# jyjblrd/Low-Cost-Mocap

Measured on AMD Instinct MI355X. Metric: triangulated 3D markers/sec at 8 cams x 16 markers, higher is better.
Workload: dtype f64

## Files before the change

### low-cost-mocap_amd/csrc/frame_bb.hip

```cpp
#include "mocap_device.hpp"
#include "kernels.hpp"
#include <cstdlib>
#include "frame_common.hpp"
#include "bb_fold.hpp"

namespace mocap {

constexpr int kBBThreads = 256;
constexpr int kBBWaves = kBBThreads / 64;
constexpr int kBBRecs = kBBThreads + 64;
constexpr int bb_cw(int C) { return C <= 8 ? 1 : 2; }
constexpr uint32_t bb_rec_bytes(int CW) { return 24u + 8u * (uint32_t)CW; }

constexpr int bb_wg_per_cu(int RL) { return RL == 48 ? 5 : 4; }
constexpr size_t kBBCacheEntry = 4;
constexpr int kBBLdsSlack = 1024;
struct BBLayout {
  size_t bxy, bxy_nx, cnt_nx, bt, rbound, seedkey, slot_key, claimw, recs, rpk, scr, scr_bytes, goff, gcnt, outslot, boff, bnb, seedgh, slot_g, cnt,
      misc, bpl, nh, hits, act, root_blob, root_cam, nact, bnl, bv, pkbase, seen, bcache, total;
  int ncache;
  __host__ __device__ static size_t al(size_t x, size_t a) { return (x + a - 1) / a * a; }
  __host__ __device__ BBLayout(int C, int M, int R, int CW, int wg_per_cu) {
    size_t o = 0;
    auto take = [&](size_t bytes, size_t a) {
// ... 553 lines not shown
        }
        const bool flag = lane < Mi && !((claimed >> lane) & 1ull);
        const unsigned long long mask = __ballot(flag);
        const int pos = __popcll(mask & ((1ull << lane) - 1ull));
        if (flag) {
          const int rr = n_roots + pos;
          if (rr < R) {
            root_cam[rr] = (uint8_t)i;
            root_blob[rr] = (uint8_t)lane;
          }
        }
        int slot = n_new;
        for (unsigned long long mm = mask; mm; slot++) {
          const int jb = __ffsll((long long)mm) - 1;
          mm &= mm - 1;
          if (lane == slot) {
            nr_cam = i;
            nr_blob = jb;
          }
        }
        n_roots += __popcll(mask);
        if (n_roots > R) {
          over = true;
          n_roots = R;
        }
      }
      if (lane == 0) {
        if (over) misc[MI_STATUS] |= MOCAP_ST_ROOT_OVERFLOW_;
        misc[MI_NROOTS] = n_roots;
      }
    } else {
      float om = 0.0f;
      for (int i = tid - 64; i < C * M; i += T - 64) {
        const int c = i / M, k = i - c * M;
        if (k < cnt[c]) {
          const float2 v = bxy[i];
          om = fmaxf(om, fmaxf(fabsf(v.x), fabsf(v.y)));
          double Bc[10];
          dlt_contribution(Bc, cv.pq(PERK ? 12 * (c * C + c) : 12 * c), (double)v.x, (double)v.y);
#pragma unroll
          for (int e = 0; e < 10; e++) bt[(size_t)i * 10 + e] = Bc[e];
        }
      }
      if (om > 0.0f) atomicMax(&misc[MI_OMAX], __float_as_int(om));
      if (tid == 64) {
        const int it = q_add(&p.q.counters[QC_NEXT_FRAME], 1);
        misc[MI_NEXT] = it < frame_count(p) ? it : -1;
      }
    }
    bb_prio<kPrioPhase>();
    __syncthreads();
    if (pre) {
      const int n_new = misc[MI_NROOTS] - n0;
      for (int idx = tid; idx < n_new * C; idx += T) {
        const int q = idx / C, c = idx - q * C;
        const int r = n0 + q, ps = bnl[q];
        if (c > (int)root_cam[r]) {
          const int n = nh_s[(size_t)ps * C + c];
          nh[(size_t)r * C + c] = (uint8_t)n;
          const uint8_t* src = hits_s + ((size_t)ps * C + c) * M;
          uint8_t* dst = hits + ((size_t)r * C + c) * M;
          for (int t = 0; t < n; t++) dst[t] = src[t];
        }
      }
      __syncthreads();
    }

    fresh_tid();
    const int nroots = misc[MI_NROOTS];
    for (int r = tid; r < nroots; r += T) {
      const int rc = root_cam[r];
      unsigned long long total = 1;
      int views = 1, na = 0;
      bool over = false;
      Packed<CW> pkb;
      pkb.clear();
      pkb.set(rc, root_blob[r]);
      uint32_t sm = 1u << rc;
      for (int c = rc + 1; c < C; c++) {
        const unsigned n = nh[(size_t)r * C + c];
        if (n > 1) act[(size_t)r * C + na++] = (uint8_t)c;
        if (n == 1) pkb.set(c, hits[((size_t)r * C + c) * M]);
        if (n) {
          sm |= 1u << c;
          views++;
          total *= n;
          if (total > (unsigned long long)p.G_cap) {
            over = true;
            total = 1;
          }
        }
      }
      if (over) atomicOr(&misc[MI_STATUS], MOCAP_ST_CAND_OVERFLOW_);
      nact[r] = (uint8_t)na;
      bv[r] = (uint8_t)views;
#pragma unroll
      for (int k = 0; k < CW; k++) pkbase[(size_t)r * CW + k] = pkb.w[k];
      if (PERK) seen[r] = (uint16_t)sm;
      rbound[r] = kInfBits;
      const uint32_t g = (views > 1 && !over) ? (uint32_t)total : 0u;
      gcnt[r] = g;
      {
        const uint8_t* a = act + (size_t)r * C;
        uint32_t pl = 1, nb = 1;
        int nl = 0;
        for (int k = 0; k < na; k++) nb *= nh[(size_t)r * C + a[k]];
        if (over) nb = 1;
        while (nl < na && (pl < (uint32_t)p.bb_pl_min || (pl < (uint32_t)p.bb_pl && nb > (uint32_t)p.bb_nb_max))) {
          const uint32_t n = nh[(size_t)r * C + a[nl++]];
          uint32_t dummy;
          pl *= n;
          divmod_small(nb, n, nb, dummy);
        }
        bpl[r] = (uint16_t)pl;
        bnl[r] = (uint8_t)nl;
        bnb[r] = g ? nb : 0u;
        seedkey[r] = 0ull;
        seedgh[r] = 0xFFFFFFFFu;
      }
    }
    for (int s = tid; s < W * RS; s += T) {
      slot_key[s] = ~0ull;
      slot_g[s] = 0xFFFFFFFFu;
    }
    if (tid == 0) misc[MI_BBCTR] = misc[MI_BBCTR2] = 0;
    __syncthreads();
    if (wave == 0) bb_prio<kPrioSerial>();
    if (wave == 0) {
      uint32_t carry = 0, bcarry = 0;
      int slots = 0;
      for (int base = 0; base < nroots; base += 64) {
        const int r = base + lane;
        const uint32_t g = r < nroots ? gcnt[r] : 0u;
        const uint32_t nb = r < nroots ? bnb[r] : 0u;
        const uint32_t incl = wave_inclusive_scan(g, lane);
        const uint32_t bincl = wave_inclusive_scan(nb, lane);
        const unsigned long long nz = __ballot(g != 0u);
        if (r < nroots) {
          goff[r] = carry + incl - g;
          boff[r] = bcarry + bincl - nb;
          outslot[r] = g ? slots + __popcll(nz & ((1ull << lane) - 1ull)) : -1;
        }
        carry += (uint32_t)__builtin_amdgcn_readlane((int)incl, 63);
        bcarry += (uint32_t)__builtin_amdgcn_readlane((int)bincl, 63);
        slots += __popcll(nz);
      }
      if (lane == 0) {
        goff[nroots] = carry;
        boff[nroots] = bcarry;
        misc[MI_NOUT] = slots;
        misc[MI_G] = misc[MI_STATUS] ? 0 : (int32_t)carry;
      }
    }
    bb_prio<kPrioPhase>();
    __syncthreads();
  }

  __device__ __forceinline__ void add_view(double (&B)[10], int c, uint32_t k, int j) const {
    if (PERK && j != c) {
      const float2 w = bxy[(size_t)c * M + k];
      double Bc[10];
      dlt_contribution(Bc, cv.base + 12 * ((size_t)j * cn() + c), (double)w.x, (double)w.y);
#pragma unroll
      for (int e = 0; e < 10; e++) B[e] = B[e] + Bc[e];
    } else {
      const double* t = bt + ((size_t)c * M + k) * 10;
#pragma unroll
      for (int e = 0; e < 10; e++) B[e] = B[e] + t[e];
    }
  }

  template <bool WITH_B>
  __device__ __forceinline__ int group_matrix(int r, uint32_t rem, int skip, double (&B)[10], Packed<CW>& pk) const {
    const int C = cn();
    const int rc = root_cam[r];
    const uint8_t* nhr = nh + (size_t)r * C;
    const uint8_t* hr = hits + (size_t)r * C * M;
    pk.clear();
    int v = 0, ka = 0;
    int j = 0;
    if (WITH_B) {
#pragma unroll
      for (int e = 0; e < 10; e++) B[e] = 0.0;
    }
    for (int c = 0; c < C; c++) {
      uint32_t k = 0xFFu;
      bool seen = false;
      if (c == rc) {
        k = root_blob[r];
        seen = true;
      } else if (c > rc) {
        const uint32_t n = nhr[c];
        seen = n != 0;
        if (n == 1) {
          k = hr[(size_t)c * M];
        } else if (n > 1) {
          if (ka >= skip) {
            uint32_t qd, dgt;
            if (rem < 8192u) divmod_tiny(rem, n, qd, dgt); else
            divmod_small(rem, n, qd, dgt);
            rem = qd;
            k = hr[(size_t)c * M + dgt];
          }
          ka++;
        }
      }
      if (k != 0xFFu) {
        if (WITH_B) add_view(B, c, k, j);
        v++;
        pk.set(c, k);
      }
      if (PERK) j += seen ? 1 : 0;
    }
    return v;
  }

  __device__ __forceinline__ void block_pk(int r, uint32_t gh, Packed<CW>& pk) const {
    const int C = cn();
#pragma unroll
    for (int k = 0; k < CW; k++) pk.w[k] = pkbase[(size_t)r * CW + k];
    const uint8_t* a = act + (size_t)r * C;
    const int na = nact[r];
    uint32_t rem = gh;
    for (int k = bnl[r]; k < na; k++) {
      const int c = a[k];
      const uint32_t n = nh[(size_t)r * C + c];
      uint32_t qd, dgt;
      if (rem < 8192u) divmod_tiny(rem, n, qd, dgt); else
      divmod_small(rem, n, qd, dgt);
      rem = qd;
      pk.set(c, hits[((size_t)r * C + c) * M + dgt]);
    }
  }
  __device__ __forceinline__ int block_matrix(int r, uint32_t gh, Packed<CW>& pk, double (&B)[10]) const {
    const int C = cn();
    block_pk(r, gh, pk);
#pragma unroll
    for (int ee = 0; ee < 10; ee++) B[ee] = 0.0;
    if constexpr (PERK) {
      const uint32_t sm = seen[r];
#pragma unroll CT > 0 ? CT : 1
      for (int c = 0; c < C; c++) {
        const uint32_t k = pk.get(c);
        if (k != 0xFFu) add_view(B, c, k, __popc(sm & ((1u << c) - 1u)));
      }
    } else {
#pragma unroll CT > 0 ? CT : 1
      for (int c = 0; c < C; c++) {
        const uint32_t k = pk.get(c);
        const double* t = bt + (size_t)(k != 0xFFu ? (uint32_t)c * (uint32_t)M + k : (uint32_t)C * (uint32_t)M) * 10;
#pragma unroll
        for (int ee = 0; ee < 10; ee++) B[ee] = B[ee] + t[ee];
      }
    }
    return (int)bv[r] - (int)bnl[r];
  }

  __device__ __forceinline__ int fetch_candidate(uint32_t lo, uint32_t i, int& r, uint32_t& gl, Packed<CW>& pk, double (&B)[10]) const {
    const int C = cn();
    const BRec rec = recs[lo];
    r = (int)(rec.rs & 0xFFu);
#pragma unroll
    for (int k = 0; k < CW; k++) pk.w[k] = rpk[(size_t)lo * CW + k];
    if (rec.rs >> 31) {
      gl = rec.gh;
    } else {
      uint32_t rem = i - (rec.rs >> 8);
      gl = rec.gh * (uint32_t)bpl[r] + rem;
      const uint8_t* a = act + (size_t)r * C;
      const int nl = bnl[r];
      for (int k = 0; k < nl; k++) {
        const int c = a[k];
        uint32_t qd, dgt;
        divmod_tiny(rem, nh[(size_t)r * C + c], qd, dgt);
        rem = qd;
        pk.set(c, hits[((size_t)r * C + c) * M + dgt]);
      }
    }
#pragma unroll
    for (int ee = 0; ee < 10; ee++) B[ee] = 0.0;
    if constexpr (PERK) {
      int j = 0;
#pragma unroll CT > 0 ? CT : 1
      for (int c = 0; c < C; c++) {
        const uint32_t k = pk.get(c);
        if (k != 0xFFu) add_view(B, c, k, j++);
      }
    } else {
#pragma unroll CT > 0 ? CT : 1
      for (int c = 0; c < C; c++) {
        const uint32_t k = pk.get(c);
        const double* t = bt + (size_t)(k != 0xFFu ? (uint32_t)c * (uint32_t)M + k : (uint32_t)C * (uint32_t)M) * 10;
#pragma unroll
        for (int ee = 0; ee < 10; ee++) B[ee] = B[ee] + t[ee];
      }
    }
    return bv[r];
  }

  __device__ void search(bool bound_tests) {
    fresh_tid();
    const int C = cn();
    (void)C;
    const int nroots = misc[MI_NROOTS];
    int32_t* ctr = &misc[MI_BBCTR];
    int32_t* ctr_other = &misc[MI_BBCTR2];
    const double inf = __builtin_huge_val();
    EigCut ec;
    {
      const double om = (double)__int_as_float(misc[MI_OMAX]);
      ec.p3max2 = p.p3max2;
      ec.o2slack = (1100.0 * 0x1p-46) * (om * om);
    }
    const double c0[3] = {p.bb_c0[0], p.bb_c0[1], p.bb_c0[2]};
    const uint32_t nblocks = boff[nroots];
    auto root_of_block = [&](uint32_t b_first_of_wave, uint32_t b) {
      return coop_last_le([&](int r) { return boff[r]; }, nroots, b_first_of_wave, b, lane);
    };
    auto push_block = [&](int r, uint32_t gh, const Packed<CW>& pk) {
      const uint32_t old = (uint32_t)atomicAdd(ctr, (int32_t)(((uint32_t)bpl[r] << 10) | 1u));
      const uint32_t slot = old & 0x3FFu;
      BRec rec;
      rec.gh = gh;
      rec.rs = (uint32_t)r | ((old >> 10) << 8);
      recs[slot] = rec;
#pragma unroll
      for (int k = 0; k < CW; k++) rpk[(size_t)slot * CW + k] = pk.w[k];
    };
    auto rec_start = [&](int k) { return (recs[k].rs & 0x7FFFFFFFu) >> 8; };
    auto root_y = [&](int r) {
      const int vf = bv[r];
      const double bound = __longlong_as_double((long long)rbound[r]);
      const double limit = bound * (double)(2 * vf) * (1.0 + 0x1p-40);
      const double limit_adj = fma(1.002, limit, (double)(2 * vf) * ec.o2slack);
      return p.p3max2c * limit_adj;
    };
    auto dropped = [&](int r, double s1, double tr) { return s1 * fma(2e-12, tr, root_y(r)) < 1.0; };
    if (bound_tests) {
      bb_prio<kPrioSeed>();
      int my_r = -1;
      uint32_t my_gh = 0;
      unsigned long long my_key = 0ull;
      Packed<CW> my_pk;
      my_pk.clear();
      for (uint32_t s0 = 0; s0 < nblocks; s0 += T) {
        const uint32_t b = s0 + (uint32_t)tid;
        if (s0 + (uint32_t)(wave * 64) >= nblocks) continue;
        const int r = root_of_block(s0 + (uint32_t)(wave * 64), b < nblocks ? b : nblocks - 1);
        if (b < nblocks) {
          const uint32_t gh = b - boff[r];
          double B[10], tr = 0.0;
          Packed<CW> pk;
          const int v = block_matrix(r, gh, pk, B);
          double s1d = __builtin_huge_val();
          float s1 = 0.0f;
          if (v >= 2) {
            s1d = eigcut_s1_shifted(B, c0, tr);
            s1 = (float)fmin(s1d, 3e38);
          }
          if (b < (uint32_t)ncache) bcache[b] = v >= 2 ? bb_fold_bound(s1d, tr) : bb_fold_inf();
          my_key = ((unsigned long long)__float_as_uint(s1) << 32) | (unsigned long long)(0xFFFFFFFFu - gh);
          my_r = r;
          my_gh = gh;
          my_pk = pk;
          atomicMax(&seedkey[r], my_key);
        }
      }
      __syncthreads();
      if (nblocks <= (uint32_t)T) {
        if (my_r >= 0 && seedkey[my_r] == my_key) {
          seedgh[my_r] = my_gh;
          push_block(my_r, my_gh, my_pk);
        }
      } else
      for (int r = tid; r < nroots; r += T) {
        if (bnb[r]) {
          const uint32_t gh = 0xFFFFFFFFu - (uint32_t)seedkey[r];
          seedgh[r] = gh;
          seedkey[r] = 0ull;
          Packed<CW> pk;
          block_pk(r, gh, pk);
          push_block(r, gh, pk);
        }
      }
      bb_prio<kPrioEval>();
      __syncthreads();
    }
    uint32_t b0 = 0;
    fresh_tid();
    while (true) {
      const uint32_t cv_ = (uint32_t)*ctr;
      const uint32_t ns = cv_ & 0x3FFu, ne = cv_ >> 10;
      const bool blocks_left = b0 < nblocks;
      const bool full = ns > (uint32_t)(kBBRecs - T);
      if (ns && (full || !blocks_left || ne >= (uint32_t)p.bb_flush)) {
        for (uint32_t i0 = 0; i0 < ne; i0 += T) {
          const uint32_t i = i0 + (uint32_t)tid;
          const bool have = i < ne;
          double e = inf, X[3] = {0, 0, 0};
          int r = 0;
          uint32_t gl = 0;
          uint32_t lo = 0;
          if (i0 + (uint32_t)(wave * 64) < ne)
            lo = (uint32_t)coop_last_le(rec_start, (int)ns, i0 + (uint32_t)(wave * 64), have ? i : ne - 1, lane);
          Packed<CW> pk;
          pk.clear();
          if (have) {
            double B[10];
            const int v = fetch_candidate(lo, i, r, gl, pk, B);
            auto obs_p = [&](int c, double& x, double& y) -> bool {
              const uint32_t k = pk.get(c);
              if (k == 0xFFu) return false;
              const float2 w = bxy[(size_t)c * M + k];
              x = (double)w.x;
              y = (double)w.y;
              return true;
            };
            const double bound = __longlong_as_double((long long)rbound[r]);
            solve_and_score<!PERK, true, F32R, false>(cv, B, v, obs_p, X, e, bound * (double)(2 * v) * (1.0 + 0x1p-40), ec);
#ifdef MOCAP_DEBUG_EIGCHECK
            if (!(e < inf)) {
              double B2[10], X2[3], e2;
#pragma unroll
              for (int ee = 0; ee < 10; ee++) B2[ee] = 0.0;
              int j2 = 0;
              for (int c = 0; c < C; c++) {
                const uint32_t k = pk.get(c);
                if (k != 0xFFu) add_view(B2, c, k, j2++);
              }
              solve_and_score<!PERK, true, F32R>(cv, B2, v, obs_p, X2, e2);
              atomicAdd(&p.status[p.n_frames], 1);
              if (e2 <= bound) printf("EIGCHECK candidate: root %d g %u bound %.17g true %.17g\n", r, gl, bound, e2);
            }
#endif
          }
          const bool fin = e < inf;
          const unsigned long long key = fin ? (unsigned long long)__double_as_longlong(e) : kInfBits;
          const uint32_t gword = (gl << 1) | ((e != e) ? 1u : 0u);
          const int ss = wave * RS + r;
          if (fin) atomicMin(&rbound[r], key);
          const bool want = have && (key < slot_key[ss] || (key == slot_key[ss] && gword < slot_g[ss]));
          if (__ballot(want)) {
            unsigned long long old = 0;
            if (want) old = atomicMin(&slot_key[ss], key);
            wave_lds_sync();
            const bool holder = want && slot_key[ss] == key;
            if (holder && old > key) slot_g[ss] = 0xFFFFFFFFu;
            wave_lds_sync();
            if (holder) atomicMin(&slot_g[ss], gword);
            wave_lds_sync();
            if (holder && slot_g[ss] == gword) store_winner(ss, X, pk);
          }
        }
        __syncthreads();
        if (tid == 0) *ctr = 0;
        {
          int32_t* t = ctr;
          ctr = ctr_other;
          ctr_other = t;
        }
        continue;
      }
      if (!blocks_left) break;
      const uint32_t b = b0 + (uint32_t)tid;
      const uint32_t bw = b0 + (uint32_t)(wave * 64);
      b0 += T;
      int r = 0;
      if (bw < nblocks) r = root_of_block(bw, b < nblocks ? b : nblocks - 1);
      bool do_push = false;
      uint32_t gh = 0;
      Packed<CW> pk;
      pk.clear();
      if (b < nblocks) {
        gh = b - boff[r];
        if (gh != seedgh[r]) {
          double B[10], tr;
          bool survive = true;
          if (bound_tests && b < (uint32_t)ncache) {
            survive = !bb_fold_dropped(bcache[b], root_y(r));
            if (survive) block_pk(r, gh, pk);
          } else if (bound_tests) {
            const int v = block_matrix(r, gh, pk, B);
            if (v >= 2) {
              const double s1 = eigcut_s1_shifted(B, c0, tr);
              survive = !dropped(r, s1, tr);
            }
          } else {
            block_pk(r, gh, pk);
          }
          do_push = survive;
#ifdef MOCAP_DEBUG_EIGCHECK
          if (!survive) {
            const double bound = __longlong_as_double((long long)rbound[r]);
            const uint32_t pl = bpl[r];
            for (uint32_t l = 0; l < pl; l++) {
              double B2[10], X2[3], e2 = inf;
              Packed<CW> pk2;
              const int v2 = group_matrix<true>(r, gh * pl + l, 0, B2, pk2);
              auto obs2 = [&](int c, double& x, double& y) -> bool {
                const uint32_t k = pk2.get(c);
                if (k == 0xFFu) return false;
                const float2 w = bxy[(size_t)c * M + k];
                x = (double)w.x;
                y = (double)w.y;
                return true;
              };
              solve_and_score<!PERK, true, F32R>(cv, B2, v2, obs2, X2, e2);
              atomicAdd(&p.status[p.n_frames + 1], 1);
              if (e2 <= bound) printf("EIGCHECK block: root %d block %u candidate %u bound %.17g true %.17g\n", r, gh, l, bound, e2);
            }
          }
#endif
        }
      }
      __syncthreads();
      if (do_push) push_block(r, gh, pk);
      __syncthreads();
    }
    wait_own_stores();
    __syncthreads();
  }

  __device__ __forceinline__ bool root_winner(int r, unsigned long long& kb, uint32_t& gw, int& wb) const {
    kb = ~0ull;
    gw = 0xFFFFFFFFu;
    wb = 0;
    for (int w = 0; w < W; w++) {
      const int s = w * RS + r;
      const unsigned long long k = slot_key[s];
      const uint32_t g = slot_g[s];
      if (k < kb || (k == kb && g < gw)) {
        kb = k;
        gw = g;
        wb = w;
      }
    }
    return kb != ~0ull;
  }

  static constexpr uint32_t kRecBytes = bb_rec_bytes(CW);
  __device__ __forceinline__ unsigned char* winner_rec(int s) const {
    return p.ws + (size_t)blockIdx.x * p.ws_stride + (size_t)(kRecBytes * (uint32_t)s);
  }
  __device__ __forceinline__ void store_winner(int s, const double (&X)[3], const Packed<CW>& pk) const {
    unsigned long long* rec = (unsigned long long*)winner_rec(s);
    if constexpr (CW == 1) {
      typedef unsigned long long rec2_t __attribute__((ext_vector_type(2)));
      const rec2_t lo = {(unsigned long long)__double_as_longlong(X[0]), (unsigned long long)__double_as_longlong(X[1])};
      const rec2_t hi = {(unsigned long long)__double_as_longlong(X[2]), pk.w[0]};
      ((rec2_t*)rec)[0] = lo;
      ((rec2_t*)rec)[1] = hi;
    } else {
#pragma unroll
      for (int k = 0; k < 3; k++) rec[k] = (unsigned long long)__double_as_longlong(X[k]);
#pragma unroll
      for (int k = 0; k < CW; k++) rec[3 + k] = pk.w[k];
    }
  }
  __device__ static __forceinline__ uint32_t row_word(uint32_t two) {
    const uint32_t x = (two & 0xFFu) | ((two & 0xFF00u) << 8);
    const uint32_t none = ((x + 0x00010001u) >> 8) & 0x00010001u;
    return x | none * 0xFF00u;
  }
  __device__ void write_point(int64_t frame, int r) const {
    const int C = cn();
    unsigned long long kb;
    uint32_t gw;
    int wv;
    if (!root_winner(r, kb, gw, wv)) return;
    const double e = kb != kInfBits ? __longlong_as_double((long long)kb)
                                    : ((gw & 1u) ? __longlong_as_double(0x7ff8000000000000ll) : __builtin_huge_val());
    const size_t o = (size_t)frame * R + outslot[r];
    const unsigned long long* rec = (const unsigned long long*)winner_rec(wv * RS + r);
    unsigned long long w[3 + CW];
#pragma unroll
    for (int k = 0; k < 3 + CW; k++) w[k] = q_ld(rec + k);
    p.err[o] = e;
    const double X[3] = {__longlong_as_double((long long)w[0]), __longlong_as_double((long long)w[1]), __longlong_as_double((long long)w[2])};
    int16_t* co = p.corr + o * C;
    if constexpr (CT == 8) {
      typedef uint32_t row_t __attribute__((ext_vector_type(4), aligned(2)));
      const uint32_t lo = (uint32_t)w[3], hi = (uint32_t)(w[3] >> 32);
      row_t v = {row_word(lo), row_word(lo >> 16), row_word(hi), row_word(hi >> 16)};
      *(row_t*)co = v;
    } else {
      for (int c = 0; c < C; c++) {
        const uint32_t k = (uint32_t)(w[3 + (CW == 1 ? 0 : c >> 3)] >> (8 * (c & 7))) & 0xFFu;
        co[c] = k == 0xFFu ? (int16_t)-1 : (int16_t)k;
      }
    }
    store_point(p, o, X);
  }
};

template <bool F32R, int CW, int CT, int ML, int RL>
__global__ __launch_bounds__(kBBThreads, bb_wg_per_cu(RL)) void frame_bb_kernel(FrameArgs p) {
  extern __shared__ __attribute__((aligned(16))) unsigned char smem[];
#define BB_STATE BBState<F32R, CW, CT, ML, RL>
#include "frame_bb_body.inc"
#undef BB_STATE
}

template <bool F32R, int CW, int CT, int ML, int RL>
__global__ __launch_bounds__(kBBThreads, bb_wg_per_cu(RL)) void frame_bb_calib_kernel(FrameArgs p) {
  extern __shared__ __attribute__((aligned(16))) unsigned char smem[];
#define BB_STATE BBState<F32R, CW, CT, ML, RL, true>
#include "frame_bb_body.inc"
#undef BB_STATE
}

int frame_bb_wg_per_cu_cap(int C, int M, int R) { return bb_wg_per_cu(bb_fixed_slots(C, M, R)); }
size_t frame_bb_ws_bytes(int) { return BBLayout::al(bb_rec_bytes(2) * (size_t)kBBWaves * 255, 256); }
static_assert(bb_wg_per_cu(48) <= kBBMaxWgPerCu && bb_wg_per_cu(64) <= kBBMaxWgPerCu && bb_wg_per_cu(0) <= kBBMaxWgPerCu, "frame_capi.hip sizes the workspace for kBBMaxWgPerCu workgroups per CU");

hipError_t launch_frame_bb(const FrameArgs& a, int grid, hipStream_t stream) {
  const size_t lds = frame_bb_lds_bytes(a.cv.C, a.M, a.K_max);
  if (!a.ws || a.ws_stride < bb_rec_bytes(bb_cw(a.cv.C)) * (size_t)kBBWaves * (size_t)frame_bb_root_slots(a.cv.C, a.M, a.K_max)) return hipErrorInvalidValue;
  const size_t nPq = a.cv.uniformK ? (size_t)12 * a.cv.C : (size_t)12 * a.cv.C * a.cv.C;
  if (a.cv.RT != a.cv.Pq + nPq || a.cv.K4 != a.cv.RT + 12 * a.cv.C || a.cv.F != a.cv.K4 + 4 * a.cv.C) return hipErrorInvalidValue;
  void (*k)(FrameArgs);
  const bool f32 = a.cv.f32_rounding != 0;
  const int fixed = bb_fixed_slots(a.cv.C, a.M, a.K_max);
  if (fixed && fixed != 48 && fixed != 64) return hipErrorInvalidValue;
  static_assert(bb_cw(8) == 1 && bb_cw(9) == 2 && bb_cw(16) == 2, "BB_PICK takes CW = 1 up to eight cameras, CW = 2 above");
#define BB_PICK(KERNEL)                                                                             \
  (fixed == 48       ? (f32 ? KERNEL<true, 1, 8, 16, 48> : KERNEL<false, 1, 8, 16, 48>)             \
   : fixed == 64     ? (f32 ? KERNEL<true, 1, 8, 16, 64> : KERNEL<false, 1, 8, 16, 64>)             \
   : a.cv.C == 8     ? (f32 ? KERNEL<true, 1, 8, 0, 0> : KERNEL<false, 1, 8, 0, 0>)                 \
   : a.cv.C <= 8     ? (f32 ? KERNEL<true, 1, 0, 0, 0> : KERNEL<false, 1, 0, 0, 0>)                 \
                     : (f32 ? KERNEL<true, 2, 0, 0, 0> : KERNEL<false, 2, 0, 0, 0>))
  k = a.cv.uniformK ? BB_PICK(frame_bb_kernel) : BB_PICK(frame_bb_calib_kernel);
#undef BB_PICK
  if (lds > 48 * 1024) {
    hipError_t e = hipFuncSetAttribute((const void*)k, hipFuncAttributeMaxDynamicSharedMemorySize, (int)lds);
    if (e != hipSuccess) return e;
  }
  hipLaunchKernelGGL(k, dim3(grid), dim3(kBBThreads), lds, stream, a);
  return hipGetLastError();
}

}
```

### low-cost-mocap_amd/csrc/mocap_device.hpp

```cpp
#pragma once
#include <hip/hip_runtime.h>
#include <stdint.h>

namespace mocap {

constexpr int kMaxCameras = 64;
constexpr int kMaxBlobs = 256;

typedef const double __attribute__((address_space(4))) * ctab_t;
__host__ __device__ inline ctab_t as_ctab(const double* p) { return (ctab_t)(uintptr_t)p; }

struct CamView {
  int C;
  int uniformK;
  int f32_rounding;
  int _pad;
  const double* Pq;
  const double* RT;
  const double* K4;
  const double* F;
  __device__ __forceinline__ ctab_t pq(size_t off) const { return as_ctab(Pq + off); }
  __device__ __forceinline__ ctab_t rt(size_t off) const { return as_ctab(RT + off); }
  __device__ __forceinline__ ctab_t k4(size_t off) const { return as_ctab(K4 + off); }
};

typedef const double __attribute__((address_space(3))) * ltab_t;
struct LdsCamView {
  int C;
  int uniformK;
  int f32_rounding;
  int _pad;
  ltab_t Pq;
  ltab_t RT;
  const double* K4;
  __device__ __forceinline__ ltab_t pq(size_t off) const { return Pq + off; }
  __device__ __forceinline__ ltab_t rt(size_t off) const { return RT + off; }
  __device__ __forceinline__ ctab_t k4(size_t off) const { return as_ctab(K4 + off); }
};

template <int CT>
struct CamViewFixed {
  const CamView& v;
  static constexpr int C = CT;
  __device__ __forceinline__ ctab_t pq(size_t off) const { return v.pq(off); }
  __device__ __forceinline__ ctab_t rt(size_t off) const { return v.rt(off); }
  __device__ __forceinline__ ctab_t k4(size_t off) const { return v.k4(off); }
};

__host__ __device__ constexpr int sidx(int i, int j) {
  return i <= j ? (i == 0 ? j : i == 1 ? 3 + j : i == 2 ? 5 + j : 9)
                : (j == 0 ? i : j == 1 ? 3 + i : j == 2 ? 5 + i : 9);
}


__device__ __forceinline__ void wait_own_stores() { asm volatile("s_waitcnt vmcnt(0)" ::: "memory"); }

__device__ __forceinline__ void block_sync_lds() {
  asm volatile("s_waitcnt lgkmcnt(0)" ::: "memory");
  __syncthreads();
}

__device__ __forceinline__ double rsqrt_pos(double d) {
  const double y = __builtin_amdgcn_rsq(d);
  const double e = fma(-(d * y), y, 1.0);
  return fma(y * e, fma(e, 0.375, 0.5), y);
}

__device__ __forceinline__ double recip_refined(double b) {
  double r = __builtin_amdgcn_rcp(b);
  r = fma(fma(-b, r, 1.0), r, r);
  r = fma(fma(-b, r, 1.0), r, r);
  return r;
}

__device__ __forceinline__ double div_by(double a, double b, double r) {
  const double q = a * r;
  return fma(fma(-b, q, a), r, q);
}

constexpr int kInvIters = 5;
constexpr int kMaxFactorisations = 32;
__device__ __forceinline__ bool smallest_eigvec4(const double (&a)[10], double (&out)[4], double lamcut, double& lam_lb) {
  const double tr = (a[0] + a[4]) + (a[7] + a[9]);
  const double floor_piv = tr * 1e-30 + 1e-300;
  double lam = 0.0, piv3 = 1.0, s1_last = 1.0, lam_last = 0.0;
  double m[10];
  for (int it = 0; it < kMaxFactorisations; it++) {
    const double r0 = rsqrt_pos(fmax(a[0] - lam, floor_piv));
    const double l10 = a[1] * r0, l20 = a[2] * r0, l30 = a[3] * r0;
    const double r1 = rsqrt_pos(fmax(fma(-l10, l10, a[4] - lam), floor_piv));
    const double l21 = fma(-l20, l10, a[5]) * r1, l31 = fma(-l30, l10, a[6]) * r1;
    const double r2 = rsqrt_pos(fmax(fma(-l21, l21, fma(-l20, l20, a[7] - lam)), floor_piv));
    const double l32 = fma(-l31, l21, fma(-l30, l20, a[8])) * r2;
    piv3 = fmax(fma(-l32, l32, fma(-l31, l31, fma(-l30, l30, a[9] - lam))), floor_piv);
    const double r3 = rsqrt_pos(piv3);
    const double m00 = r0, m11 = r1, m22 = r2, m33 = r3;
    const double m10 = -(l10 * m00) * m11;
    const double m21 = -(l21 * m11) * m22;
    const double m32 = -(l32 * m22) * m33;
    const double m20 = -fma(l21, m10, l20 * m00) * m22;
    const double m31 = -fma(l32, m21, l31 * m11) * m33;
    const double m30 = -fma(l32, m20, fma(l31, m10, l30 * m00)) * m33;
    m[0] = m00; m[1] = m10; m[2] = m20; m[3] = m30; m[4] = m11; m[5] = m21; m[6] = m31; m[7] = m22;
    m[8] = m32; m[9] = m33;
    const double w00 = fma(m00, m00, fma(m10, m10, fma(m20, m20, m30 * m30)));
    const double w11 = fma(m11, m11, fma(m21, m21, m31 * m31));
    const double w22 = fma(m22, m22, m32 * m32);
    const double w33 = m33 * m33;
    const double s1 = (w00 + w11) + (w22 + w33);
    if (it == 0 && s1 * fma(2e-12, tr, lamcut) < 1.0) return false;
    s1_last = s1;
    lam_last = lam;
    const double w01 = fma(m10, m11, fma(m20, m21, m30 * m31));
    const double w02 = fma(m20, m22, m30 * m32);
    const double w03 = m30 * m33;
    const double w12 = fma(m21, m22, m31 * m32);
    const double w13 = m31 * m33;
    const double w23 = m32 * m33;
    const double sd = fma(w00, w00, fma(w11, w11, fma(w22, w22, w33 * w33)));
    const double so = fma(w01, w01, fma(w02, w02, fma(w03, w03, fma(w12, w12, fma(w13, w13, w23 * w23)))));
    const double s2 = fma(2.0, so, sd);
    const double s1sq = s1 * s1;
    if (!(s1sq - s2 > 1e-3 * s1sq)) break;
    const double disc = fmax(3.0 * fma(4.0, s2, -s1sq), 1e-300);
    const double den = fma(disc, __builtin_amdgcn_rsq(disc), s1);
    lam = fma(4.0 - 0x1p-18, __builtin_amdgcn_rcp(den), lam);
  }
  double x0 = m[3], x1 = m[6], x2 = m[8], x3 = m[9];
#pragma unroll
  for (int k = 1; k < kInvIters; k++) {
    const double y0 = (m[0] * x0) * piv3;
    const double y1 = fma(m[1], x0, m[4] * x1) * piv3;
    const double y2 = fma(m[2], x0, fma(m[5], x1, m[7] * x2)) * piv3;
    const double y3 = fma(m[3], x0, fma(m[6], x1, fma(m[8], x2, m[9] * x3))) * piv3;
    x0 = fma(m[0], y0, fma(m[1], y1, fma(m[2], y2, m[3] * y3)));
    x1 = fma(m[4], y1, fma(m[5], y2, m[6] * y3));
    x2 = fma(m[7], y2, m[8] * y3);
    x3 = m[9] * y3;
  }
  out[0] = x0;
  out[1] = x1;
  out[2] = x2;
  out[3] = x3;
  lam_lb = fma(1.0 - 1e-5, __builtin_amdgcn_rcp(s1_last), lam_last) - 2e-12 * tr;
  return true;
}

__device__ __forceinline__ double eigcut_s1(const double (&a)[10], double& tr) {
  tr = (a[0] + a[4]) + (a[7] + a[9]);
  const double floor_piv = tr * 1e-30 + 1e-300;
  const double r0 = rsqrt_pos(fmax(a[0], floor_piv));
  const double l10 = a[1] * r0, l20 = a[2] * r0, l30 = a[3] * r0;
  const double r1 = rsqrt_pos(fmax(fma(-l10, l10, a[4]), floor_piv));
  const double l21 = fma(-l20, l10, a[5]) * r1, l31 = fma(-l30, l10, a[6]) * r1;
  const double r2 = rsqrt_pos(fmax(fma(-l21, l21, fma(-l20, l20, a[7])), floor_piv));
  const double l32 = fma(-l31, l21, fma(-l30, l20, a[8])) * r2;
  const double r3 = rsqrt_pos(fmax(fma(-l32, l32, fma(-l31, l31, fma(-l30, l30, a[9]))), floor_piv));
  const double m10 = -(l10 * r0) * r1;
  const double m21 = -(l21 * r1) * r2;
  const double m32 = -(l32 * r2) * r3;
  const double m20 = -fma(l21, m10, l20 * r0) * r2;
  const double m31 = -fma(l32, m21, l31 * r1) * r3;
  const double m30 = -fma(l32, m20, fma(l31, m10, l30 * r0)) * r3;
  const double w00 = fma(r0, r0, fma(m10, m10, fma(m20, m20, m30 * m30)));
  const double w11 = fma(r1, r1, fma(m21, m21, m31 * m31));
  const double w22 = fma(r2, r2, m32 * m32);
  return (w00 + w11) + (w22 + r3 * r3);
}

__device__ __forceinline__ double eigcut_s1_shifted(const double (&a)[10], const double (&c)[3], double& tr) {
  double b[10];
  b[0] = a[0]; b[1] = a[1]; b[2] = a[2]; b[4] = a[4]; b[5] = a[5]; b[7] = a[7];
  b[3] = fma(a[0], c[0], fma(a[1], c[1], fma(a[2], c[2], a[3])));
  b[6] = fma(a[1], c[0], fma(a[4], c[1], fma(a[5], c[2], a[6])));
  b[8] = fma(a[2], c[0], fma(a[5], c[1], fma(a[7], c[2], a[8])));
  b[9] = fma(c[0], b[3] + a[3], fma(c[1], b[6] + a[6], fma(c[2], b[8] + a[8], a[9])));
  double tr1;
  const double s1 = eigcut_s1(b, tr1);
  const double c2 = fma(c[0], c[0], fma(c[1], c[1], fma(c[2], c[2], 1.0)));
  tr = tr1 + 2.0 * c2 * ((a[0] + a[4]) + (a[7] + a[9]));
  return s1;
}

struct EigCut {
  double p3max2 = 0.0;
  double o2slack = 0.0;
};

template <class Tab>
__device__ __forceinline__ void dlt_contribution(double (&Bc)[10], Tab P, double x, double y) {
  double ra[4], rb[4];
#pragma unroll
  for (int k = 0; k < 4; k++) {
    ra[k] = y * P[8 + k] - P[4 + k];
    rb[k] = P[k] - x * P[8 + k];
  }
#pragma unroll
  for (int i = 0; i < 4; i++)
#pragma unroll
    for (int j = i; j < 4; j++) Bc[sidx(i, j)] = fma(ra[i], ra[j], rb[i] * rb[j]);
}

template <class Tab>
__device__ __forceinline__ void dlt_accumulate(double (&B)[10], Tab P, double x, double y) {
  double Bc[10];
  dlt_contribution(Bc, P, x, y);
#pragma unroll
  for (int e = 0; e < 10; e++) B[e] = B[e] + Bc[e];
}

template <bool F32R, class Tab>
__device__ __forceinline__ void reproject_sq(Tab RT, ctab_t K4, const double (&X)[3], double ox,
                                             double oy, double& du2, double& dv2) {
  double x = RT[0] * X[0] + RT[1] * X[1] + RT[2] * X[2] + RT[9];
  double y = RT[3] * X[0] + RT[4] * X[1] + RT[5] * X[2] + RT[10];
  double z = RT[6] * X[0] + RT[7] * X[1] + RT[8] * X[2] + RT[11];
  z = z != 0.0 ? div_by(1.0, z, recip_refined(z)) : 1.0;
  x *= z;
  y *= z;
  double pu = x * K4[0] + K4[2];
  double pv = y * K4[1] + K4[3];
  if (F32R) {
    pu = (double)(float)pu;
    pv = (double)(float)pv;
  }
  const double du = ox - pu, dv = oy - pv;
  du2 = du * du;
  dv2 = dv * dv;
}

template <bool UNIFORM_K, bool PAIRWISE, bool F32R, int BATCH = 1, class View, class Obs2>
__device__ __forceinline__ void score_point(const View& cv, int v, Obs2&& obs2, const double (&X)[3], double& err,
                                            double limit);

template <bool UNIFORM_K, bool PAIRWISE, bool F32R, bool DEPTH_CUT = true, int BATCH = 1, class View, class Obs2>
__device__ __forceinline__ void solve_and_score(const View& cv, double (&B)[10], int v, Obs2&& obs2,
                                                double (&X)[3], double& err,
                                                double limit = __builtin_huge_val(), const EigCut& ec = EigCut{}) {
  const double inf = __builtin_huge_val();
  const bool cut = ec.p3max2 > 0.0;
  const double limit_adj = fma(1.002, limit, (double)(2 * v) * ec.o2slack);
  double vec[4], lam_lb;
  if (!smallest_eigvec4(B, vec, cut ? ec.p3max2 * limit_adj : inf, lam_lb)) {
    X[0] = X[1] = X[2] = 0.0;
    err = inf;
    return;
  }
  const double rw = recip_refined(vec[3]);
  X[0] = div_by(vec[0], vec[3], rw);
  X[1] = div_by(vec[1], vec[3], rw);
  X[2] = div_by(vec[2], vec[3], rw);
  if (cut && DEPTH_CUT) {
    double Xp[3] = {X[0], X[1], X[2]};
    if (F32R) {
      Xp[0] = (double)(float)X[0];
      Xp[1] = (double)(float)X[1];
      Xp[2] = (double)(float)X[2];
    }
    const double n2 = fma(Xp[0], Xp[0], fma(Xp[1], Xp[1], fma(Xp[2], Xp[2], 1.0)));
    double zmax2 = 1e-14 * (n2 * ec.p3max2);
    if constexpr (BATCH > 1) {
      const int C = cv.C;
      for (int c0 = 0; c0 < C; c0 += BATCH) {
        unsigned long long rw[BATCH];
#pragma unroll
        for (int u = 0; u < BATCH; u++) rw[u] = obs2.raw(c0 + u < C ? c0 + u : C - 1);
#pragma unroll
        for (int u = 0; u < BATCH; u++) {
          double ox, oy;
          if (c0 + u < C && obs2.decode(rw[u], ox, oy)) {
            const auto RT = cv.rt(12 * (c0 + u));
            const double z = fma(RT[6], Xp[0], fma(RT[7], Xp[1], fma(RT[8], Xp[2], RT[11])));
            zmax2 = fmax(zmax2, z * z);
          }
        }
      }
    } else {
      for (int c = 0; c < cv.C; c++) {
        double ox, oy;
        if (obs2(c, ox, oy)) {
          const auto RT = cv.rt(12 * c);
          const double z = fma(RT[6], Xp[0], fma(RT[7], Xp[1], fma(RT[8], Xp[2], RT[11])));
          zmax2 = fmax(zmax2, z * z);
        }
      }
    }
    if (lam_lb * n2 > zmax2 * limit_adj) {
      err = inf;
      return;
    }
  }
  score_point<UNIFORM_K, PAIRWISE, F32R, BATCH>(cv, v, obs2, X, err, limit);
}

__device__ __forceinline__ void solve_point(double (&B)[10], double (&X)[3]) {
  double vec[4], lam_lb;
  smallest_eigvec4(B, vec, __builtin_huge_val(), lam_lb);
  const double rw = recip_refined(vec[3]);
  X[0] = div_by(vec[0], vec[3], rw);
  X[1] = div_by(vec[1], vec[3], rw);
  X[2] = div_by(vec[2], vec[3], rw);
}

template <bool UNIFORM_K, bool PAIRWISE, bool F32R, int BATCH, class View, class Obs2>
__device__ __forceinline__ void score_point(const View& cv, int v, Obs2&& obs2, const double (&X)[3], double& err,
                                            double limit) {
  const int C = cv.C;
  double Xp[3] = {X[0], X[1], X[2]};
  if (F32R) {
    Xp[0] = (double)(float)X[0];
    Xp[1] = (double)(float)X[1];
    Xp[2] = (double)(float)X[2];
  }
  const bool pw = PAIRWISE && v == C && 2 * C >= 8;
  const int C4 = C & ~3;
  double seq = 0.0, r[8] = {0, 0, 0, 0, 0, 0, 0, 0};
  int j = 0;
  for (int c0 = 0; c0 < C4; c0 += 4) {
    if (!(seq <= limit)) continue;
    unsigned long long rw[4] = {0, 0, 0, 0};
    if constexpr (BATCH > 1) {
#pragma unroll
      for (int u = 0; u < 4; u++) rw[u] = obs2.raw(c0 + u);
    }
#pragma unroll
    for (int u = 0; u < 4; u++) {
      double x, y;
      bool seen;
      if constexpr (BATCH > 1)
        seen = obs2.decode(rw[u], x, y);
      else
        seen = obs2(c0 + u, x, y);
      if (seen) {
        double du2, dv2;
        reproject_sq<F32R>(cv.rt(12 * (c0 + u)), cv.k4(4 * (UNIFORM_K ? 0 : j)), Xp, x, y, du2, dv2);
        seq = seq + du2;
        seq = seq + dv2;
        if (PAIRWISE) {
          r[2 * u] = r[2 * u] + du2;
          r[2 * u + 1] = r[2 * u + 1] + dv2;
        }
        j++;
      }
    }
  }
  double spw = ((r[0] + r[1]) + (r[2] + r[3])) + ((r[4] + r[5]) + (r[6] + r[7]));
  for (int c = C4; c < C; c++) {
    double x, y;
    if (obs2(c, x, y)) {
      double du2, dv2;
      reproject_sq<F32R>(cv.rt(12 * c), cv.k4(4 * (UNIFORM_K ? 0 : j)), Xp, x, y, du2, dv2);
      seq = seq + du2;
      seq = seq + dv2;
      if (PAIRWISE) {
        spw = spw + du2;
        spw = spw + dv2;
      }
      j++;
    }
  }
  err = (seq <= limit) ? (pw ? spw : seq) / (double)(2 * v) : __builtin_huge_val();
}

template <bool UNIFORM_K, bool PAIRWISE, bool F32R, int BATCH = 1, bool DEPTH_CUT = true, class View, class Obs1, class Obs2>
__device__ __forceinline__ int triangulate_and_score(const View& cv, Obs1&& obs1, Obs2&& obs2,
                                                     double (&X)[3], double& err,
                                                     double limit_e = __builtin_huge_val(), const EigCut& ec = EigCut{}) {
  const int C = cv.C;
  double B[10] = {0, 0, 0, 0, 0, 0, 0, 0, 0, 0};
  int v = 0;
  if constexpr (BATCH > 1) {
    for (int c0 = 0; c0 < C; c0 += BATCH) {
      unsigned long long rw[BATCH];
#pragma unroll
      for (int u = 0; u < BATCH; u++) rw[u] = obs1.raw(c0 + u < C ? c0 + u : C - 1);
#pragma unroll
      for (int u = 0; u < BATCH; u++) {
        double x, y;
        if (c0 + u < C && obs1.decode(rw[u], x, y)) {
          dlt_accumulate(B, cv.pq(UNIFORM_K ? (size_t)12 * (c0 + u) : 12 * ((size_t)v * C + (c0 + u))), x, y);
          v++;
        }
      }
    }
  } else {
    for (int c = 0; c < C; c++) {
      double x, y;
      if (obs1(c, x, y)) {
        dlt_accumulate(B, cv.pq(UNIFORM_K ? (size_t)12 * c : 12 * ((size_t)v * C + c)), x, y);
        v++;
      }
    }
  }
  if (v <= 1) return v;
  solve_and_score<UNIFORM_K, PAIRWISE, F32R, DEPTH_CUT, BATCH>(cv, B, v, obs2, X, err, limit_e * (double)(2 * v) * (1.0 + 0x1p-40), ec);
  return v;
}

template <bool PAIRWISE, bool F32R, class Contrib, class Obs2>
__device__ __forceinline__ int triangulate_and_score_tab(const CamView& cv, Contrib&& contrib, Obs2&& obs2,
                                                         double (&X)[3], double& err,
                                                         double limit_e = __builtin_huge_val(), const EigCut& ec = EigCut{}) {
  const int C = cv.C;
  double B[10] = {0, 0, 0, 0, 0, 0, 0, 0, 0, 0};
  int v = 0;
  for (int c = 0; c < C; c++) v += contrib(c, B) ? 1 : 0;
  if (v <= 1) return v;
  solve_and_score<true, PAIRWISE, F32R>(cv, B, v, obs2, X, err, limit_e * (double)(2 * v) * (1.0 + 0x1p-40), ec);
  return v;
}

}
```

Measured before the change: 599.3 million.

## Use LDS-only barriers in BB search and peel first score group

Replaces several __syncthreads calls in the branch-and-bound search loop with a barrier that waits only on LDS/scalar counters (lgkmcnt) rather than draining outstanding global memory operations. It also adds a waitcnt at search entry and a BORN variant of score_point that peels the first 4-camera group so the pairwise accumulators are initialized by assignment instead of adding to zero. The aim is to cut barrier stalls on vmem traffic and a few adds per candidate. The risk is that global stores or atomics are no longer ordered at those barriers, which could break correctness if other threads rely on seeing them.

```diff
diff --git a/low-cost-mocap_amd/csrc/frame_bb.hip b/low-cost-mocap_amd/csrc/frame_bb.hip
--- a/low-cost-mocap_amd/csrc/frame_bb.hip
+++ b/low-cost-mocap_amd/csrc/frame_bb.hip
@@ -879,6 +879,7 @@
     fresh_tid();
     const int C = cn();
     (void)C;
+    __builtin_amdgcn_s_waitcnt(0x0F70);
     const int nroots = misc[MI_NROOTS];
     int32_t* ctr = &misc[MI_BBCTR];
     int32_t* ctr_other = &misc[MI_BBCTR2];
@@ -943,7 +944,7 @@
           atomicMax(&seedkey[r], my_key);
         }
       }
-      __syncthreads();
+      block_sync_lds_only();
       if (nblocks <= (uint32_t)T) {
         if (my_r >= 0 && seedkey[my_r] == my_key) {
           seedgh[my_r] = my_gh;
@@ -961,7 +962,7 @@
         }
       }
       bb_prio<kPrioEval>();
-      __syncthreads();
+      block_sync_lds_only();
     }
     uint32_t b0 = 0;
     fresh_tid();
@@ -994,7 +995,7 @@
               return true;
             };
             const double bound = __longlong_as_double((long long)rbound[r]);
-            solve_and_score<!PERK, true, F32R, false>(cv, B, v, obs_p, X, e, bound * (double)(2 * v) * (1.0 + 0x1p-40), ec);
+            solve_and_score<!PERK, true, F32R, false, 1, true>(cv, B, v, obs_p, X, e, bound * (double)(2 * v) * (1.0 + 0x1p-40), ec);
 #ifdef MOCAP_DEBUG_EIGCHECK
             if (!(e < inf)) {
               double B2[10], X2[3], e2;
@@ -1029,7 +1030,7 @@
             if (holder && slot_g[ss] == gword) store_winner(ss, X, pk);
           }
         }
-        __syncthreads();
+        block_sync_lds_only();
         if (tid == 0) *ctr = 0;
         {
           int32_t* t = ctr;
@@ -1090,9 +1091,9 @@
 #endif
         }
       }
-      __syncthreads();
+      block_sync_lds_only();
       if (do_push) push_block(r, gh, pk);
-      __syncthreads();
+      block_sync_lds_only();
     }
     wait_own_stores();
     __syncthreads();
diff --git a/low-cost-mocap_amd/csrc/mocap_device.hpp b/low-cost-mocap_amd/csrc/mocap_device.hpp
--- a/low-cost-mocap_amd/csrc/mocap_device.hpp
+++ b/low-cost-mocap_amd/csrc/mocap_device.hpp
@@ -1,6 +1,7 @@
 #pragma once
 #include <hip/hip_runtime.h>
 #include <stdint.h>
+#include <type_traits>
 
 namespace mocap {
 
@@ -59,6 +60,8 @@
   asm volatile("s_waitcnt lgkmcnt(0)" ::: "memory");
   __syncthreads();
 }
+
+__device__ __forceinline__ void block_sync_lds_only() { asm volatile("s_waitcnt lgkmcnt(0)\n\ts_barrier" ::: "memory"); }
 
 __device__ __forceinline__ double rsqrt_pos(double d) {
   const double y = __builtin_amdgcn_rsq(d);
@@ -229,11 +232,11 @@
   dv2 = dv * dv;
 }
 
-template <bool UNIFORM_K, bool PAIRWISE, bool F32R, int BATCH = 1, class View, class Obs2>
+template <bool UNIFORM_K, bool PAIRWISE, bool F32R, int BATCH = 1, bool BORN = false, class View, class Obs2>
 __device__ __forceinline__ void score_point(const View& cv, int v, Obs2&& obs2, const double (&X)[3], double& err,
                                             double limit);
 
-template <bool UNIFORM_K, bool PAIRWISE, bool F32R, bool DEPTH_CUT = true, int BATCH = 1, class View, class Obs2>
+template <bool UNIFORM_K, bool PAIRWISE, bool F32R, bool DEPTH_CUT = true, int BATCH = 1, bool BORN = false, class View, class Obs2>
 __device__ __forceinline__ void solve_and_score(const View& cv, double (&B)[10], int v, Obs2&& obs2,
                                                 double (&X)[3], double& err,
                                                 double limit = __builtin_huge_val(), const EigCut& ec = EigCut{}) {
@@ -290,7 +293,7 @@
       return;
     }
   }
-  score_point<UNIFORM_K, PAIRWISE, F32R, BATCH>(cv, v, obs2, X, err, limit);
+  score_point<UNIFORM_K, PAIRWISE, F32R, BATCH, BORN>(cv, v, obs2, X, err, limit);
 }
 
 __device__ __forceinline__ void solve_point(double (&B)[10], double (&X)[3]) {
@@ -302,7 +305,7 @@
   X[2] = div_by(vec[2], vec[3], rw);
 }
 
-template <bool UNIFORM_K, bool PAIRWISE, bool F32R, int BATCH, class View, class Obs2>
+template <bool UNIFORM_K, bool PAIRWISE, bool F32R, int BATCH, bool BORN, class View, class Obs2>
 __device__ __forceinline__ void score_point(const View& cv, int v, Obs2&& obs2, const double (&X)[3], double& err,
                                             double limit) {
   const int C = cv.C;
@@ -316,31 +319,71 @@
   const int C4 = C & ~3;
   double seq = 0.0, r[8] = {0, 0, 0, 0, 0, 0, 0, 0};
   int j = 0;
-  for (int c0 = 0; c0 < C4; c0 += 4) {
-    if (!(seq <= limit)) continue;
-    unsigned long long rw[4] = {0, 0, 0, 0};
-    if constexpr (BATCH > 1) {
-#pragma unroll
-      for (int u = 0; u < 4; u++) rw[u] = obs2.raw(c0 + u);
-    }
-#pragma unroll
-    for (int u = 0; u < 4; u++) {
-      double x, y;
-      bool seen;
-      if constexpr (BATCH > 1)
-        seen = obs2.decode(rw[u], x, y);
-      else
-        seen = obs2(c0 + u, x, y);
-      if (seen) {
-        double du2, dv2;
-        reproject_sq<F32R>(cv.rt(12 * (c0 + u)), cv.k4(4 * (UNIFORM_K ? 0 : j)), Xp, x, y, du2, dv2);
-        seq = seq + du2;
-        seq = seq + dv2;
-        if (PAIRWISE) {
-          r[2 * u] = r[2 * u] + du2;
-          r[2 * u + 1] = r[2 * u + 1] + dv2;
-        }
-        j++;
+  if constexpr (BORN) {
+    auto group = [&](int c0, auto first) {
+      constexpr bool FIRST = decltype(first)::value;
+      unsigned long long rw[4] = {0, 0, 0, 0};
+      if constexpr (BATCH > 1) {
+#pragma unroll
+        for (int u = 0; u < 4; u++) rw[u] = obs2.raw(c0 + u);
+      }
+#pragma unroll
+      for (int u = 0; u < 4; u++) {
+        double x, y;
+        bool seen;
+        if constexpr (BATCH > 1)
+          seen = obs2.decode(rw[u], x, y);
+        else
+          seen = obs2(c0 + u, x, y);
+        double du2 = 0.0, dv2 = 0.0;
+        if (seen) {
+          reproject_sq<F32R>(cv.rt(12 * (c0 + u)), cv.k4(4 * (UNIFORM_K ? 0 : j)), Xp, x, y, du2, dv2);
+          seq = seq + du2;
+          seq = seq + dv2;
+          if (PAIRWISE && !FIRST) {
+            r[2 * u] = r[2 * u] + du2;
+            r[2 * u + 1] = r[2 * u + 1] + dv2;
+          }
+          j++;
+        }
+        if (PAIRWISE && FIRST) {
+          r[2 * u] = du2;
+          r[2 * u + 1] = dv2;
+        }
+      }
+    };
+    if (C4 > 0) group(0, std::true_type{});
+    for (int c0 = 4; c0 < C4; c0 += 4) {
+      if (!(seq <= limit)) continue;
+      group(c0, std::false_type{});
+    }
+  } else {
+    for (int c0 = 0; c0 < C4; c0 += 4) {
+      if (!(seq <= limit)) continue;
+      unsigned long long rw[4] = {0, 0, 0, 0};
+      if constexpr (BATCH > 1) {
+#pragma unroll
+        for (int u = 0; u < 4; u++) rw[u] = obs2.raw(c0 + u);
+      }
+#pragma unroll
+      for (int u = 0; u < 4; u++) {
+        double x, y;
+        bool seen;
+        if constexpr (BATCH > 1)
+          seen = obs2.decode(rw[u], x, y);
+        else
+          seen = obs2(c0 + u, x, y);
+        if (seen) {
+          double du2, dv2;
+          reproject_sq<F32R>(cv.rt(12 * (c0 + u)), cv.k4(4 * (UNIFORM_K ? 0 : j)), Xp, x, y, du2, dv2);
+          seq = seq + du2;
+          seq = seq + dv2;
+          if (PAIRWISE) {
+            r[2 * u] = r[2 * u] + du2;
+            r[2 * u + 1] = r[2 * u + 1] + dv2;
+          }
+          j++;
+        }
       }
     }
   }
```

New measurement: 613.4 million (median of 6 runs). 2.4% higher.
